# Varkalandar/raysnail

Hardware: AMD Instinct MI355X
Metric: Msamples/s (whole node) + ms/frame, RTIOW-13.1 scene 800x500x64spp (higher is better)
Workload: dtype f64; 1 GPU; rtow_13_1 balls_scene(seed 7)+light, 800x500, 64 spp, depth 8; width=800, height=500, spp=64, depth=8, split=rows, lanes=default, frames_in_flight=default, samples_per_frame=25600000

## Files before the change

raysnail_amd/csrc/rs_cam_cand.h:

```cpp
#pragma once
#include <math.h>
#include <stdint.h>

#if defined(__HIPCC__) || defined(__CUDACC__)
#define RS_CC_HD __host__ __device__
#else
#define RS_CC_HD
#endif

namespace rs {

constexpr uint32_t kCandMax = 8;
constexpr uint32_t kCandEmpty = 0xFFFFu;
constexpr uint32_t kCandOverflow = 0xFFFEu;
constexpr uint32_t kCandMaxEntries = 65534u;
constexpr int kCandStack = 32;

struct CandCam {
    double o[3];
    double lb[3], hf[3], vf[3];
    double R;
    double rho;
    double inv_w, inv_h, h;
    int ok;
// ... 33 lines not shown
    const double slack = 1.0 + 0x1p-40;
    c.R = fabs(aperture) * 0.5 * sqrt((hu2 > vu2 ? hu2 : vu2) + huvu) * slack;
    c.rho = sqrt(hf2 / (4.0 * w * w) + vf2 / (4.0 * h * h) + hfvf / (2.0 * w * h)) * slack;
    c.inv_w = 1.0 / w; c.inv_h = 1.0 / h; c.h = h;
    c.ok = cand_finite(c.R) && cand_finite(c.rho);
    return c;
}

RS_CC_HD inline CandBeam cand_beam(const CandCam& c, uint32_t x, uint32_t y) {
    CandBeam b;
    const double u = ((double)x + 0.5) * c.inv_w, v = (c.h - 1.5 - (double)y) * c.inv_h;
    double l2 = 0.0;
    for (int k = 0; k < 3; ++k) {
        b.o[k] = c.o[k];
        b.d[k] = c.lb[k] + u * c.hf[k] + v * c.vf[k] - c.o[k];
        l2 += b.d[k] * b.d[k];
    }
    b.len = sqrt(l2);
    b.inv_len = 1.0 / b.len;
    b.inv_len2 = 1.0 / l2;
    b.R = c.R; b.rho = c.rho;
    b.ok = c.ok && cand_finite(l2) && l2 > 0.0 && cand_finite(b.inv_len2);
    b.b[0] = c.rho - c.R;
    b.b[1] = c.R + c.rho;
    b.wide = 0;
    for (int piece = 0; piece < 2; ++piece) {
        const double k = b.b[piece] * b.inv_len;
        if (!(fabs(k) <= 0.99)) { b.wide = 1; b.kf[piece] = 0.0; continue; }
        b.kf[piece] = k * b.inv_len / sqrt(1.0 - k * k);
    }
    return b;
}

RS_CC_HD inline bool cand_sphere(const CandBeam& b, const double c[3], double r, double* along = nullptr) {
    const double w[3] = {c[0] - b.o[0], c[1] - b.o[1], c[2] - b.o[2]};
    const double w1 = fabs(w[0]) + fabs(w[1]) + fabs(w[2]);
    const double p = (w[0] * b.d[0] + w[1] * b.d[1] + w[2] * b.d[2]) * b.inv_len2;
    if (along) *along = p;
    if (!b.ok || b.wide) return true;
    r = fabs(r);
    const double reach = w1 + b.R + r;
    r = sqrt(r * r + 0x1p-40 * reach * reach);
    if (!(r - r == 0.0)) return true;
    const double cx = w[1] * b.d[2] - w[2] * b.d[1], cy = w[2] * b.d[0] - w[0] * b.d[2], cz = w[0] * b.d[1] - w[1] * b.d[0];
    const double h = sqrt(cx * cx + cy * cy + cz * cz) * b.inv_len;
    for (int piece = 0; piece < 2; ++piece) {
        const double bb = b.b[piece];
        const double aa = piece == 0 ? r + b.R : r - b.R;
        double s = p + h * b.kf[piece];
        if (piece == 0) s = s < 0.0 ? 0.0 : s > 1.0 ? 1.0 : s;
        else s = s < 1.0 ? 1.0 : s;
        if (!(s - s == 0.0)) return true;
        const double q[3] = {w[0] - s * b.d[0], w[1] - s * b.d[1], w[2] - s * b.d[2]};
        const double dist = sqrt(q[0] * q[0] + q[1] * q[1] + q[2] * q[2]);
        const double g = dist - (aa + bb * s);
        const double slack = 0x1p-30 * (w1 + r + b.R + s * (b.len + b.R + b.rho));
        if (!(g > slack)) return true;
    }
    return false;
}

struct CandList {
    uint32_t e[kCandMax];
    double along[kCandMax];
    uint32_t n;
};
// ... 18 lines not shown
```

raysnail_amd/csrc/rs_host.cpp:

```cpp
#include <hip/hip_runtime.h>

#include <algorithm>
#include <atomic>
#include <chrono>
#include <functional>
#include <cmath>
#include <cstdio>
#include <cstdlib>
#include <cstring>
#include <memory>
#include <new>
#include <stdexcept>
#include <string>
#include <vector>

#include "../../include/raysnail_hip.h"
#include "rs_host_util.h"
#include "rs_internal.h"
#include "rs_layout.h"

using namespace rs;

namespace {

// ... 670 lines not shown
    DScene& d = s->hs.ds;
    d.limg = nullptr;
    d.limg_bytes = 0;
    std::memset(d.limg_off, 0, sizeof(d.limg_off));
    if (s->scene_mode != kSmNest0 && s->scene_mode != kSmNest2) return;
    if (d.root4 < 0 || !d.ref_order || s->stack_need + (int)kLeafBatch > stack_lds(s->scene_mode)) return;
    const uint32_t cap = kLimgMax;
#ifdef RS_DEV_KNOBS
    if (std::getenv("RS_NO_LIMG")) return;
#endif
    const void* const* fields[LT_COUNT] = {
        (const void* const*)&d.nodes4, (const void* const*)&d.pbox, (const void* const*)&d.pclass,
        (const void* const*)&d.prims, (const void* const*)&d.spheres, (const void* const*)&d.rects,
        (const void* const*)&d.boxes, (const void* const*)&d.quadrics, (const void* const*)&d.csgs,
        (const void* const*)&d.xforms, (const void* const*)&d.tf_fwd, (const void* const*)&d.tf_inv};
    std::vector<char> img;
    for (int t = 0; t < LT_COUNT; ++t) {
        const size_t fo = (size_t)((const char*)fields[t] - (const char*)&d);
        img.resize((img.size() + 15) & ~(size_t)15);
        d.limg_off[t] = (uint32_t)img.size();
        for (const Blob& b : s->hs.blobs)
            if (b.field_off == fo) img.insert(img.end(), b.bytes.begin(), b.bytes.end());
        if (img.size() > cap) return;
    }
    img.resize((img.size() + 15) & ~(size_t)15);
    if (img.size() > cap) return;
    d.limg_bytes = (uint32_t)img.size();
    Blob b;
    b.field_off = (size_t)((const char*)&d.limg - (const char*)&d);
    b.bytes = std::move(img);
    s->hs.blobs.push_back(std::move(b));
}

void upload_replica(rs_scene* s, int device) {
    std::unique_ptr<Replica> R(new Replica());
    R->device = device;
    HIP_OK(hipSetDevice(device));
    R->ds = s->hs.ds;
    for (const Blob& b : s->hs.blobs) {
        void* p = nullptr;
        HIP_OK(hipMalloc(&p, b.bytes.size()));
        R->dev.push_back(p);
        HIP_OK(hipMemcpy(p, b.bytes.data(), b.bytes.size(), hipMemcpyHostToDevice));
        std::memcpy((char*)&R->ds + b.field_off, &p, sizeof(void*));
    }
    HIP_OK(hipMalloc((void**)&R->d_ds, sizeof(DScene)));
    std::memset(&R->uploaded, 0xff, sizeof(DScene));
    HIP_OK(hipStreamCreateWithFlags(&R->stream, hipStreamNonBlocking));
#ifdef RS_DEV_KNOBS
    if (const char* e = std::getenv("RS_PAD_STREAMS"))
        for (int k = std::atoi(e); k > 0; --k) {
            hipStream_t st;
            HIP_OK(hipStreamCreateWithFlags(&st, hipStreamNonBlocking));
            R->pad_streams.push_back(st);
        }
#endif
    hipDeviceProp_t prop;
    HIP_OK(hipGetDeviceProperties(&prop, device));
    R->n_cu = prop.multiProcessorCount;
    R->mem_total = (uint64_t)prop.totalGlobalMem;
    HIP_OK(wf_occupancy(s->scene_mode, &R->ext_bpc, &R->shade_bpc));
    s->reps.push_back(std::move(R));
}

void build(rs_scene* s) {
    if (s->committed) throw Error(RS_E_STATE, "scene already committed");
    s->hs = HostScene();
    for (uint32_t h : s->world) if (s->nest_depth(h) > RS_MAX_NEST) throw Error(RS_E_UNSUPPORTED, "object nesting deeper than the GPU path supports");
    for (uint32_t h : s->lights) if (s->nest_depth(h) > RS_MAX_NEST) throw Error(RS_E_UNSUPPORTED, "light nesting deeper than the GPU path supports");

    std::vector<DMaterial> mats;
    for (const rs_material_desc& d : s->mdesc) {
        DMaterial m;
        std::memset(&m, 0, sizeof(m));
        m.kind = d.kind; m.tex_kind = d.texture.kind; m.tex_data = d.texture.data; m.glass = d.glass;
        m.k_specular = d.k_specular;
        m.mix_a = d.mix_a; m.mix_b = d.mix_b;
        for (int i = 0; i < 4; ++i) { m.even[i] = d.texture.even[i]; m.odd[i] = d.texture.odd[i]; }
        m.tex_scale = d.texture.scale;
        m.enter_refractive = 1.0 / d.refractive;
        m.outer_refractive = d.refractive;
        m.exponent = d.exponent; m.multiplier = d.multiplier; m.mix_p = d.mix_p;
        const rs_material_desc* e = &d;
        for (int k = 0; k < 64 && e->kind == RS_MAT_MIXED; ++k) e = &s->mdesc[e->mix_a];
        m.phong_factor = e->phong_factor; m.phong_exponent = e->phong_exponent;
        mats.push_back(m);
    }
    DMaterial dm;
    std::memset(&dm, 0, sizeof(dm));
    dm.kind = RS_MAT_LAMBERTIAN; dm.tex_kind = RS_TEX_SOLID;
    for (int i = 0; i < 4; ++i) dm.even[i] = 1.0f;
    dm.enter_refractive = dm.outer_refractive = 1.0; dm.multiplier = 1.0; dm.phong_exponent = 1;
    const int32_t default_mat = (int32_t)mats.size();
    mats.push_back(dm);
// ... 279 lines not shown
            s->tree_depth = depth4;
            s->n_nodes = n4.size();
            s->stack_need = stack_need4_ref(n4, r4);
        }
    }
    d.stack_need = s->stack_need;
    d.moving = 0;
    for (const DSphere& sp : spheres)
        if (sp.v[0] != 0.0 || sp.v[1] != 0.0 || sp.v[2] != 0.0) d.moving = 1;
    d.stk_ovf = nullptr;
    stage(s, d.prims, prims);
    stage(s, d.spheres, spheres);
    stage(s, d.lprim, leaves.prims);
    s->n_leaf_entries = leaves.prims.size();
    if (s->scene_mode == kSmSpheres) {
        std::vector<DSphere> lsph(s->objs.size());
        std::memset(lsph.data(), 0, lsph.size() * sizeof(DSphere));
        for (size_t h = 0; h < s->objs.size(); ++h)
            if (s->objs[h].kind == PK_SPHERE) lsph[h] = spheres[prims[h].idx];
        if (lsph.size() * sizeof(DSphere) > 0xFFFFFFFFull) throw Error(RS_E_INVALID, "scene too large: sphere array over 4 GiB");
        if (d.moving) {
            stage(s, d.lsph, lsph);
        } else {
            std::vector<DSphereS> lsphs(lsph.size());
            for (size_t h = 0; h < lsph.size(); ++h) {
                for (int k = 0; k < 3; ++k) lsphs[h].c[k] = lsph[h].c[k];
                lsphs[h].r = lsph[h].r;
                if (s->objs[h].kind == PK_SPHERE && lsph[h].r * lsph[h].r != lsph[h].r2)
                    throw Error(RS_E_INVALID, "sphere radius_squared is not radius * radius");
            }
            stage(s, d.lsphs, lsphs);
        }
    }
    if (s->scene_mode == kSmFlat) {
        std::vector<LTri> ltri(leaves.prims.size());
        std::memset(ltri.data(), 0, ltri.size() * sizeof(LTri));
        for (size_t e = 0; e < ltri.size(); ++e) {
            const DPrim& P = prims[leaves.prims[e]];
            ltri[e].kind = (double)P.kind;
            if (P.kind != PK_TRIANGLE) continue;
            const DTri& T = tris[P.idx];
            for (int k = 0; k < 3; ++k) ltri[e].p0[k] = T.p0[k];
            ltri[e].a = T.a; ltri[e].b = T.b; ltri[e].c = T.c; ltri[e].d = T.d; ltri[e].e = T.e; ltri[e].f = T.f;
        }
        if (ltri.size() * sizeof(LTri) > 0xFFFFFFFFull) throw Error(RS_E_INVALID, "scene too large: leaf triangle array over 4 GiB");
        stage(s, d.ltri, ltri);
    }
    stage(s, d.rects, rects);
    stage(s, d.boxes, boxes);
    stage(s, d.quadrics, quads);
    stage(s, d.tris, tris);
    stage(s, d.csgs, csgs);
    stage(s, d.xforms, xforms);
    stage(s, d.tf_fwd, tf_f);
    stage(s, d.tf_inv, tf_i);
    stage(s, d.mats, mats);
    stage(s, d.media, media);
    d.has_media = media.empty() ? 0 : 1;
    std::vector<DPerlin> dper;
    std::vector<double> tf64;
    std::vector<int32_t> ti32;
    for (const HPerlin& hp : s->perlins) {
        DPerlin x;
        std::memset(&x, 0, sizeof(x));
        x.point_count = (int32_t)hp.d.point_count; x.vector = hp.d.vector; x.smooth = hp.d.smooth; x.type = hp.d.type;
        x.depth = (int32_t)hp.d.depth; x.scale = hp.d.scale;
// ... 1904 lines not shown
```

raysnail_amd/csrc/rs_internal.h:

```cpp
#pragma once
#include <hip/hip_runtime.h>
#include <stdint.h>
#include "rs_layout.h"
#include "rs_cam_cand.h"

namespace rs {

constexpr int kBlock = 256;
constexpr int kStackMax = 24;
constexpr int kStackMin = 16;
constexpr uint32_t kLeafBatch = 8;
constexpr uint32_t kMaxLanes = 4;
constexpr uint32_t kMaxSlots = 4;
constexpr int kMaxFrames = 64;

enum SceneMode { kSmGeneric = 0, kSmSpheres = 1, kSmFlat = 2, kSmNest0 = 3, kSmNest2 = 4, kSmMarch = 5 };
constexpr bool generic_mode(int sm) { return sm == kSmGeneric || sm == kSmMarch; }
constexpr int march_of(int sm) { return sm == kSmMarch ? 1 : 0; }
constexpr int nest_of(int sm) { return sm == kSmNest0 ? 0 : sm == kSmNest2 ? 2 : generic_mode(sm) ? RS_MAX_NEST : 0; }
constexpr int rich_of(int sm) { return generic_mode(sm) ? 1 : 0; }
constexpr bool streaming_mode(int sm) { return sm == kSmSpheres || sm == kSmNest0 || sm == kSmNest2; }
constexpr int stack_lds(int sm) { return generic_mode(sm) ? kStackMax : kStackMin; }
static_assert(4u * ((uint32_t)stack_lds(kSmNest0) * kBlock * 4u + kLimgMax) <= 160u * 1024u, "LDS image budget");
static_assert(4u * ((uint32_t)stack_lds(kSmNest2) * kBlock * 4u + kLimgMax) <= 160u * 1024u, "LDS image budget");

struct SceneRef {
    const DScene* host;
    const DScene* dev;
};
#if defined(RS_NO_FLAT_DYN) || defined(RS_TRAV_STATS)
inline bool flat_dyn(const SceneRef&) { return false; }
#else
inline bool flat_dyn(const SceneRef& s) { return s.host->root4 >= 0; }
#endif
#ifdef RS_NO_FLAT_LAMB
inline bool flat_lamb(const SceneRef&) { return false; }
#else
// ... 58 lines not shown
hipError_t launch_probe_shade(const SceneRef& s, const double* rows, uint32_t n, uint64_t key_base, double* out, int sm,
                              hipStream_t st);
hipError_t launch_probe_camera(const DCamera& c, const PathParams& p, const uint32_t* xys, uint32_t n, int centres,
                               double* out, int sm, hipStream_t st);
hipError_t launch_path_mega(const SceneRef& s, const DCamera& c, const PathParams& p, int sm, double* rad,
                            unsigned long long* seg_counters, uint32_t max_blocks, hipStream_t st);
hipError_t launch_wf_gen(const DCamera& c, const PathParams& p, const WfState& w, uint64_t item0, uint32_t n, double* rad,
                         hipStream_t st);
hipError_t launch_wf_extend(const SceneRef& s, const WfState& w, uint32_t bounce, uint32_t blocks, int sm, hipStream_t st);
hipError_t launch_wf_shade(const SceneRef& s, const WfState& w, uint32_t bounce, uint32_t depth, uint64_t n_items, double* rad,
                           uint32_t blocks, int sm, hipStream_t st);

constexpr int kWfsClasses = 5;
#ifndef RS_CNT_PAD
#define RS_CNT_PAD 32
#endif
constexpr uint32_t kCntPad = RS_CNT_PAD;
constexpr int kCntStat0 = 8;
constexpr uint32_t kStatLines = 8;
constexpr uint32_t kWfsStride = (kCntStat0 + kStatLines) * kCntPad;
__host__ __device__ constexpr uint32_t cix(int slot) { return (uint32_t)slot * kCntPad; }
constexpr int kCntFront = 6, kCntBack = 7;
constexpr int kExtAll = 0, kExtCarried = 1, kExtCamera = 2;
constexpr bool ext_split(int sm) { return sm == kSmNest2 || sm == kSmSpheres; }
#ifndef RS_CAM_FUSE
#define RS_CAM_FUSE 1
#endif
constexpr bool cam_fused(int sm, int part) { return RS_CAM_FUSE && sm == kSmSpheres && part == kExtCamera; }
#ifndef RS_CAM_CAND
#define RS_CAM_CAND 1
#endif
constexpr bool cam_cand(int sm, int part) { return RS_CAM_CAND && sm == kSmSpheres && part == kExtCamera; }
hipError_t launch_cam_cand_build(const SceneRef& s, const DCamera& c, const PathParams& p, uint4* cand, hipStream_t st);
hipError_t launch_wfs_extend(const SceneRef& s, const DCamera& c, const PathParams& p, const WfState& w,
                             QEnt* const* queues, uint32_t it, const InjParams& inj, double* rad, uint32_t blocks,
                             int part, int sm, hipStream_t st, hipEvent_t ev0 = nullptr, hipEvent_t ev1 = nullptr);
hipError_t launch_wfs_finish(const SceneRef& s, const WfState& w, uint32_t it, uint32_t depth, double* rad, uint32_t blocks,
                             int sm, hipStream_t st);
hipError_t launch_wfs_shade_all(const SceneRef& s, const WfState& w, QEnt* const* queues, uint32_t class_mask,
                                uint32_t it, uint32_t depth, double* rad, uint32_t blocks, bool split, int sm,
                                hipStream_t st);
hipError_t wf_occupancy(int sm, int* extend_blocks_per_cu, int* shade_blocks_per_cu);
hipError_t launch_combine(float* acc, const float* nw, uint64_t n, float p, hipStream_t st);
hipError_t launch_noise(const float* px, int w, int h, float t, uint8_t* redo, unsigned int* minmax_bits,
                        unsigned long long* count, hipStream_t st);
hipError_t launch_probe_hit(const SceneRef& s, const double* rays, uint32_t n, double tmin, double tmax, double* out, int sm,
                            hipStream_t st);
hipError_t launch_features(const SceneRef& s, const DCamera& c, const PathParams& p, uint32_t max_specular, float* out_albedo,
                           float* out_normal, unsigned long long* seg_counter, int sm, uint32_t max_blocks, hipStream_t st);
hipError_t launch_denoise(const float* beauty, const float* albedo, const float* normal, uint32_t width, uint32_t height,
                          uint32_t levels, const float* ic, float inv_n, float inv_d, int gamma, float* out, float* work,
                          hipStream_t st);
hipError_t launch_pass_moments(const float* const* frames, uint32_t n_frames, uint32_t n_pix, int gamma, float* mean,
                               float* var, hipStream_t st);
hipError_t launch_denoise_var(const float* beauty, const float* var, const float* albedo, const float* normal,
                              uint32_t width, uint32_t height, uint32_t levels, float k_color, float inv_n, float inv_d,
                              int gamma, float* out, float* out_var, float* work, hipStream_t st);
hipError_t launch_pass_robust(const float* const* frames, uint32_t n_frames, uint32_t n_pix, int gamma, float trim,
                              float* mean, float* var, uint8_t* trimmed, hipStream_t st);
hipError_t launch_moments_update(float* acc, float* m2, const float* const* frames, uint32_t n_frames, uint32_t n_pix,
                                 int gamma, hipStream_t st);
hipError_t launch_moments_resolve(const float* acc, const float* m2, uint32_t n_pix, int gamma, float* mean, float* var,
                                  hipStream_t st);
hipError_t launch_adaptive_mask(const float* acc, const float* m2, const uint8_t* base, uint32_t width, uint32_t height,
                                uint32_t min_n, uint32_t max_n, float tol2, float floor, uint32_t radius, uint8_t* mask,
                                unsigned int* counters, hipStream_t st, uint32_t row_begin, uint32_t row_end,
// ... 8 lines not shown
```

raysnail_amd/csrc/rs_kernels.hip:

```cpp
#include <cstdlib>
#include <type_traits>

#include <hip/hip_ext.h>

#include "rs_device.h"
#include "rs_internal.h"
#include "rs_gen_perm.h"

#define RS_PASTE_(a, b) a##b
#define RS_PASTE(a, b) RS_PASTE_(a, b)
#if !defined(RS_TU)
#define RS_TU_COMMON 1
#define RS_TU_MODES 1
#define RS_TU_SUFFIX
#elif RS_TU < 0
#define RS_TU_COMMON 1
#define RS_TU_MODES 0
#define RS_TU_SUFFIX _c
#elif RS_TU == 6
#define RS_TU_COMMON 0
#define RS_TU_MODES 0
#define RS_TU_SUFFIX _6
#else
#define RS_TU_COMMON 0
// ... 1265 lines not shown

constexpr int kClasses = kWfsClasses;
constexpr int kClsLight = 6;

constexpr int ext_min_waves(int sm, bool lobj = false, int part = kExtAll) {
    if (sm == kSmSpheres) return 5;
    return sm == kSmNest2 ? (lobj ? 3 : 2) : 4;
}

extern __shared__ uint4 s_limg[];
__device__ __forceinline__ void lds_fill(const DScene& Sv) {
    const uint32_t nq = Sv.limg_bytes >> 4;
    const uint4* __restrict__ src = (const uint4*)Sv.limg;
    for (uint32_t q = threadIdx.x; q < nq; q += kBlock) s_limg[q] = src[q];
    __syncthreads();
}
__device__ __forceinline__ void lds_scene(const DScene* __restrict__ Sp, DScene& Sv, bool fill = true) {
    Sv = *Sp;
    if (fill) lds_fill(Sv);
    const char* b = (const char*)s_limg;
    Sv.nodes4 = (const DNode4*)(b + Sv.limg_off[LT_NODES4]);
    Sv.pclass = (const uint8_t*)(b + Sv.limg_off[LT_PCLASS]);
    Sv.pbox = (const DBox64*)(b + Sv.limg_off[LT_PBOX]);
    Sv.prims = (const DPrim*)(b + Sv.limg_off[LT_PRIMS]);
    Sv.spheres = (const DSphere*)(b + Sv.limg_off[LT_SPHERES]);
    Sv.rects = (const DRect*)(b + Sv.limg_off[LT_RECTS]);
    Sv.boxes = (const DBox*)(b + Sv.limg_off[LT_BOXES]);
    Sv.quadrics = (const DQuadric*)(b + Sv.limg_off[LT_QUADRICS]);
    Sv.csgs = (const DCsg*)(b + Sv.limg_off[LT_CSGS]);
    Sv.xforms = (const DXform*)(b + Sv.limg_off[LT_XFORMS]);
    Sv.tf_fwd = (const DMat34*)(b + Sv.limg_off[LT_TF_FWD]);
    Sv.tf_inv = (const DMat34*)(b + Sv.limg_off[LT_TF_INV]);
}
template <int SM, bool OVF, int PART, bool LOBJ>
__global__ __launch_bounds__(kBlock, ext_min_waves(SM, LOBJ, PART)) void k_wfs_extend(const DScene* __restrict__ Sp, WfState W,
                                                                          QEnt* const* __restrict__ queues, uint32_t it,
                                                                          double* __restrict__ rad, DCamera C, PathParams P,
                                                                          InjParams I) {
    DScene Sv;
    if constexpr (LOBJ) lds_scene(Sp, Sv, false);
    const DScene& S = LOBJ ? Sv : *Sp;
    __shared__ int stk_all[stack_lds(SM) * kBlock];
    const StkT<OVF, stack_lds(SM)> stk = make_stk<OVF, stack_lds(SM)>(S, stk_all);
    constexpr bool kTop = SM == kSmSpheres && kLTop > 0;
    uint32_t* cnt = W.counts + (size_t)it * kWfsStride;
    const uint32_t nf = cnt[cix(kCntFront)];
    const uint32_t n_old = PART == kExtCamera ? 0u : nf + cnt[cix(kCntBack)];
    const uint32_t n = n_old + (PART == kExtCarried ? 0u : I.n_new);
    if (PART != kExtCamera && blockIdx.x == 0 && threadIdx.x == 0) cnt[0] = n_old;
    const WfSet& cur = W.set[it & 1];
    constexpr bool kFuse = cam_fused(SM, PART);
    constexpr bool kCand = cam_cand(SM, PART);
    const uint32_t base0 = blockIdx.x * kBlock;
    for (uint32_t base = base0; base < n; base += gridDim.x * kBlock) {
        const uint32_t j = base + threadIdx.x;
        const bool gen = PART == kExtCamera || (PART == kExtAll && j >= n_old);
        const uint32_t i = gen ? nf + (j - n_old) : j < nf ? j : W.cap - 1u - (j - nf);
        int cls = -1, qbp = 0;
        int fcls = -1;
        double qt = 0.0;
        bool live = false;
        Ray r;
        Rng rng;
        uint32_t item = 0;
        [[maybe_unused]] uint32_t pl = 0;
        if (j < n) {
            if (gen) {
                uint64_t g, key;
                inj_sample(I, P, j - n_old, g, key, item);
                live = camera_sample(C, P, key, g, r, rng, kCand ? &pl : nullptr);
                if (!live) put_rad(rad, item, 0.0, 0.0, 0.0);
            } else {
                r = load_ray(cur, i, W.tagw);
                live = true;
            }
        }
        if constexpr (LOBJ)
            if (base == base0) lds_fill(S);
        if constexpr (kTop)
            if (base == base0) {
                const uint32_t nq = (uint32_t)S.ltop * (sizeof(DNode4) / 16);
                const uint4* __restrict__ src = (const uint4*)S.nodes4;
                for (uint32_t q = threadIdx.x; q < nq; q += kBlock) ((uint4*)s_top4)[q] = src[q];
                __syncthreads();
            }
        if (live) {
            double bend = RS_INF;
            constexpr bool kT = SM == kSmSpheres;
            int bp = -1;
            bool walk = true;
            if constexpr (kCand) {
                if (I.cand) {
                    const i4v rv = gld<i4v>(I.cand, pl * 16u);
                    uint4 rec = make_uint4((uint32_t)rv.x, (uint32_t)rv.y, (uint32_t)rv.z, (uint32_t)rv.w);
                    if ((rec.x & 0xFFFFu) != kCandOverflow) {
                        const RayC rc = ray_consts(r);
                        double best = RS_INF, be = RS_INF;
                        bool tie = false;
                        TravStat st;
                        for (uint32_t k = 0; k < kCandMax; ++k) {
                            const uint32_t e = rec.x & 0xFFFFu;
                            if (e == kCandEmpty) break;
                            rec.x = (rec.x >> 16) | (rec.y << 16); rec.y = (rec.y >> 16) | (rec.z << 16);
                            rec.z = (rec.z >> 16) | (rec.w << 16); rec.w = (rec.w >> 16) | 0xFFFF0000u;
                            st.leaf();
                            test_sphere_leaf<true>(S, ld_sphere_s(S.lsphs, (int)e), (int)e, r, rc, 0.0001, best, be, bp, &tie);
                        }
                        if (!tie) {
                            walk = false;
                            st.store();
                            bend = best;
                            if (bp >= 0 && S.lprim) bp = S.lprim[bp];
                        }
                    }
                }
            }
            if (walk) bp = traverse<SM, StkT<OVF, stack_lds(SM)>, LOBJ, kT, kTop>(S, r, 0.0001, bend, stk);
            V3 add;
            bool done = true;
            if (bp < 0) {
                add = background(S, r);
            } else {
                cls = (int)S.pclass[bp];
                if (cls == kClsLight) {
                    Hit h;
                    int mi;
                    if (SM == kSmSpheres) {
                        const DPrim Pr = S.prims[bp];
                        sphere_rec_at(S.spheres[Pr.idx], Pr.mat, r, bend, h);
                        mi = Pr.mat;
                    } else {
                        if (S.prims[bp].kind != PK_XFORM) {
                            HitT ht;
                            Obj<0, 0>::hit_t(S, bp, r, 0.0001, bend, ht);
                            h.p = ht.p;
                            mi = S.prims[bp].mat;
                        } else {
                            finish_hit<SM, true>(S, bp, r, 0.0001, bend, h);
                            mi = h.mat;
                        }
                    }
                    add = emission<0>(S, S.mats[mi >= 0 ? mi : S.default_mat], h);
                    cls = -1;
                } else {
                    qbp = bp;
                    qt = bend;
                    if (kFuse && (cls == 0 || cls == 1 || cls == 3)) {
                        fcls = cls;
// ... 684 lines not shown
                                  float* out_albedo, float* out_normal, unsigned long long* seg_counter,
                                  uint32_t max_blocks, hipStream_t st) {
    const uint32_t N = p.sqrt_spp * p.sqrt_spp;
    const uint32_t ppw = 64 / (N < 64 ? (N ? N : 1u) : 64u);
    const uint64_t groups = ((uint64_t)p.n_pix_local + ppw - 1) / ppw;
    const uint64_t blocks = std::min<uint64_t>((groups + kBlock / 64 - 1) / (kBlock / 64), max_blocks);
    if (!blocks) return hipSuccess;
    if (max_specular == 0)
        hipLaunchKernelGGL(k_features<SM>, dim3((uint32_t)blocks), dim3(kBlock), 0, st, s.dev, c, p,
                           reinterpret_cast<float4*>(out_albedo), reinterpret_cast<float4*>(out_normal), seg_counter);
    else
        hipLaunchKernelGGL(k_features_spec<SM>, dim3((uint32_t)blocks), dim3(kBlock), 0, st, s.dev, c, p, max_specular,
                           reinterpret_cast<float4*>(out_albedo), reinterpret_cast<float4*>(out_normal), seg_counter);
    return hipGetLastError();
}
#if !defined(RS_TU) || RS_TU == 5
hipError_t features_march(const SceneRef& s, const DCamera& c, const PathParams& p, uint32_t max_specular, float* out_albedo,
                          float* out_normal, unsigned long long* seg_counter, uint32_t max_blocks, hipStream_t st) {
    return features_launch<kSmMarch>(s, c, p, max_specular, out_albedo, out_normal, seg_counter, max_blocks, st);
}
#endif
#if !defined(RS_TU) || RS_TU == 6
hipError_t features_march(const SceneRef& s, const DCamera& c, const PathParams& p, uint32_t max_specular, float* out_albedo,
                          float* out_normal, unsigned long long* seg_counter, uint32_t max_blocks, hipStream_t st);
hipError_t launch_features(const SceneRef& s, const DCamera& c, const PathParams& p, uint32_t max_specular, float* out_albedo,
                           float* out_normal, unsigned long long* seg_counter, int sm, uint32_t max_blocks, hipStream_t st) {
    if (sm == kSmMarch) return features_march(s, c, p, max_specular, out_albedo, out_normal, seg_counter, max_blocks, st);
    return features_launch<kSmGeneric>(s, c, p, max_specular, out_albedo, out_normal, seg_counter, max_blocks, st);
}
#endif
#endif

#if !defined(RS_TU) || RS_TU == 1
__global__ __launch_bounds__(kBlock) void k_cam_cand_build(const DScene* __restrict__ Sp, DCamera C, PathParams P,
                                                           uint4* __restrict__ cand) {
    const uint32_t pl = blockIdx.x * kBlock + threadIdx.x;
    if (pl >= P.n_pix_local) return;
    const DScene& S = *Sp;
    const uint32_t x = pl % P.width, y = P.row_begin + (pl / P.width) * P.row_step;
    const CandCam cc = cand_camera(C.origin, C.lb, C.hf, C.vf, C.hu, C.vu, C.aperture, P.width, P.height);
    const CandBeam b = cand_beam(cc, x, y);
    CandList l;
    cand_list_init(l);
    if (!b.ok || S.root4 < 0) {
        l.n = kCandMax + 1;
    } else {
        int stk[kCandStack];
        int sp = 0, node = S.root4;
        while (node >= 0 && !cand_list_overflow(l)) {
            const DNode4& N = S.nodes4[node];
            int next = -1;
            for (int k = 0; k < 4; ++k) {
                const int c = N.child[k];
                if (c == INT32_MIN) continue;
                const double lo[3] = {(double)N.lo_x[k], (double)N.lo_y[k], (double)N.lo_z[k]};
                const double hi[3] = {(double)N.hi_x[k], (double)N.hi_y[k], (double)N.hi_z[k]};
                const double ctr[3] = {0.5 * (lo[0] + hi[0]), 0.5 * (lo[1] + hi[1]), 0.5 * (lo[2] + hi[2])};
                const double ex = hi[0] - lo[0], ey = hi[1] - lo[1], ez = hi[2] - lo[2];
                const double rad = 0.5 * sqrt(ex * ex + ey * ey + ez * ez) * (1.0 + 0x1p-40);
                if (!cand_sphere(b, ctr, rad)) continue;
                if (c < 0) {
                    const DSphere sp_ = ld_sphere_s(S.lsphs, ~c);
                    double along;
                    if (cand_sphere(b, sp_.c, sp_.r, &along)) cand_list_add(l, (uint32_t)~c, along);
                } else if (next < 0) {
                    next = c;
                } else if (sp < kCandStack) {
                    stk[sp++] = c;
                } else {
                    l.n = kCandMax + 1;
                }
            }
            if (next < 0 && sp > 0) next = stk[--sp];
            node = next;
        }
    }
    uint32_t w[4];
    cand_list_pack(l, w);
    cand[pl] = make_uint4(w[0], w[1], w[2], w[3]);
}

hipError_t launch_cam_cand_build(const SceneRef& s, const DCamera& c, const PathParams& p, uint4* cand, hipStream_t st) {
    const uint32_t blocks = (p.n_pix_local + kBlock - 1) / kBlock;
    if (!blocks) return hipSuccess;
    hipLaunchKernelGGL(k_cam_cand_build, dim3(blocks), dim3(kBlock), 0, st, s.dev, c, p, cand);
    return hipGetLastError();
}
#endif

#define RS_SM_LAUNCHERS(X)                                                                                     \
    X(hipError_t, probe_sample, (const SceneRef& s, const DCamera& c, const PathParams& p, uint32_t x, uint32_t y,  \
                                 uint32_t s0, uint32_t n, double* out, hipStream_t st), (s, c, p, x, y, s0, n, out, st)) \
    X(hipError_t, path_mega, (const SceneRef& s, const DCamera& c, const PathParams& p, double* rad,              \
                              unsigned long long* seg_counters, uint32_t max_blocks, hipStream_t st),             \
      (s, c, p, rad, seg_counters, max_blocks, st))                                                            \
    X(hipError_t, wf_extend, (const SceneRef& s, const WfState& w, uint32_t bounce, uint32_t blocks, hipStream_t st), \
      (s, w, bounce, blocks, st))                                                                              \
    X(hipError_t, wf_shade, (const SceneRef& s, const WfState& w, uint32_t bounce, uint32_t depth, uint64_t n_items,  \
                             double* rad, uint32_t blocks, hipStream_t st), (s, w, bounce, depth, n_items, rad, blocks, st)) \
    X(hipError_t, wf_occupancy, (int* e, int* sh), (e, sh))                                                    \
    X(hipError_t, probe_shade, (const SceneRef& s, const double* rows, uint32_t n, uint64_t key_base, double* out,  \
                                hipStream_t st), (s, rows, n, key_base, out, st))                               \
    X(hipError_t, probe_camera, (const DCamera& c, const PathParams& p, const uint32_t* xys, uint32_t n, int centres, \
                                 double* out, hipStream_t st), (c, p, xys, n, centres, out, st))
#define RS_SORTED_LAUNCHERS(X)                                                                                 \
    X(hipError_t, wfs_extend, (const SceneRef& s, const DCamera& c, const PathParams& p, const WfState& w,       \
                               QEnt* const* queues, uint32_t it, const InjParams& inj, double* rad, uint32_t blocks, \
                               int part, hipStream_t st, hipEvent_t ev0, hipEvent_t ev1),                        \
      (s, c, p, w, queues, it, inj, rad, blocks, part, st, ev0, ev1))                                                  \
    X(hipError_t, wfs_finish, (const SceneRef& s, const WfState& w, uint32_t it, uint32_t depth, double* rad,        \
                               uint32_t blocks, hipStream_t st), (s, w, it, depth, rad, blocks, st))              \
    X(hipError_t, wfs_shade_all, (const SceneRef& s, const WfState& w, QEnt* const* queues, uint32_t class_mask, \
// ... 287 lines not shown
```

raysnail_amd/csrc/rs_layout.h:

```cpp
#pragma once
#include <stdint.h>

#define RS_MAX_NEST 4

namespace rs {

enum PrimKind : int32_t {
    PK_SPHERE = 0,
    PK_RECT = 1,
    PK_BOX = 2,
    PK_QUADRIC = 3,
    PK_TRIANGLE = 4,
    PK_AND = 5,
    PK_SUB = 6,
    PK_XFORM = 7,
    PK_MEDIUM = 8,
    PK_RAYMARCH = 9,
};

struct DPrim {
    int32_t kind;
    int32_t idx;
    int32_t mat;
    int32_t aux;
};

struct DSphere {
    double c[3];
    double r;
    double r2;
    double v[3];
};

struct alignas(32) DSphereS {
// ... 115 lines not shown
    const LTri* ltri;
    const DRect* rects;
    const DBox* boxes;
    const DQuadric* quadrics;
    const DTri* tris;
    const DCsg* csgs;
    const DXform* xforms;
    const DMat34* tf_fwd;
    const DMat34* tf_inv;
    const DMaterial* mats;
    const DMedium* media;
    const DPerlin* perlins;
    const DImage* images;
    const double* tex_f64;
    const int32_t* tex_i32;
    const uint8_t* tex_u8;
    const int32_t* lights;
    int32_t* stk_ovf;
    const void* limg;
    uint32_t limg_bytes;
    uint32_t limg_off[LT_COUNT];
    int32_t n_lights;
    int32_t root;
    int32_t default_mat;
    int32_t ref_order;
    int32_t root4;
    int32_t uv;
    int32_t has_media;
    int32_t stack_need;
    int32_t moving;
    int32_t ltop;
    int32_t lamb_only;
    float bg_lo[4], bg_hi[4];
};

#ifndef RS_LTOP
#define RS_LTOP 85
#endif
constexpr int kLTop = RS_LTOP;


struct DCamera {
    double origin[3], lb[3], hf[3], vf[3], hu[3], vu[3];
    double aperture, shutter;
};

}
```

Baseline: 5138 Msamples/s.

## Add precomputed light-directed candidate grid to skip BVH traversal for light rays

Builds a uniform 3D grid over the sphere scene. For each cell, a conservative beam (cell ball toward the single spherical light) is walked through the BVH once at upload, storing up to eight candidate spheres per cell. During extension of carried (bounce) rays whose origin cell is valid and whose direction points into the light's cone, only the candidate list is tested instead of a full traversal. It falls back to traversal on overflow or ties. This adds a per-ray membership test, grid memory and a build kernel, and only helps rays aimed at the light.

```diff
diff --git a/raysnail_amd/csrc/rs_cam_cand.h b/raysnail_amd/csrc/rs_cam_cand.h
--- a/raysnail_amd/csrc/rs_cam_cand.h
+++ b/raysnail_amd/csrc/rs_cam_cand.h
@@ -89,6 +89,32 @@
     return b;
 }
 
+RS_CC_HD inline CandBeam cand_beam_ball(const double O[3], double R, const double F[3], double rho) {
+    CandBeam b;
+    double l2 = 0.0;
+    bool fin = cand_finite(R) && cand_finite(rho);
+    for (int k = 0; k < 3; ++k) {
+        b.o[k] = O[k];
+        b.d[k] = F[k] - O[k];
+        l2 += b.d[k] * b.d[k];
+        fin = fin && cand_finite(O[k]) && cand_finite(F[k]);
+    }
+    b.len = sqrt(l2);
+    b.inv_len = 1.0 / b.len;
+    b.inv_len2 = 1.0 / l2;
+    b.R = fabs(R); b.rho = fabs(rho);
+    b.ok = fin && cand_finite(l2) && l2 > 0.0 && cand_finite(b.inv_len2);
+    b.b[0] = b.rho - b.R;
+    b.b[1] = b.R + b.rho;
+    b.wide = 0;
+    for (int piece = 0; piece < 2; ++piece) {
+        const double k = b.b[piece] * b.inv_len;
+        if (!(fabs(k) <= 0.99)) { b.wide = 1; b.kf[piece] = 0.0; continue; }
+        b.kf[piece] = k * b.inv_len / sqrt(1.0 - k * k);
+    }
+    return b;
+}
+
 RS_CC_HD inline bool cand_sphere(const CandBeam& b, const double c[3], double r, double* along = nullptr) {
     const double w[3] = {c[0] - b.o[0], c[1] - b.o[1], c[2] - b.o[2]};
     const double w1 = fabs(w[0]) + fabs(w[1]) + fabs(w[2]);
diff --git a/raysnail_amd/csrc/rs_host.cpp b/raysnail_amd/csrc/rs_host.cpp
--- a/raysnail_amd/csrc/rs_host.cpp
+++ b/raysnail_amd/csrc/rs_host.cpp
@@ -726,6 +726,13 @@
     s->hs.blobs.push_back(std::move(b));
 }
 
+bool light_cand_scene(const rs_scene* s, const DScene& d) {
+    return light_cand(s->scene_mode, kExtCarried) && d.moving == 0 && d.root4 >= 0 && !s->ref_order &&
+           s->objs.size() <= kCandMaxEntries && s->stack_need <= kCandStack && s->lights.size() == 1;
+}
+
+bool try_malloc(void** p, size_t bytes);
+
 void upload_replica(rs_scene* s, int device) {
     std::unique_ptr<Replica> R(new Replica());
     R->device = device;
@@ -754,6 +761,17 @@
     R->n_cu = prop.multiProcessorCount;
     R->mem_total = (uint64_t)prop.totalGlobalMem;
     HIP_OK(wf_occupancy(s->scene_mode, &R->ext_bpc, &R->shade_bpc));
+    if (R->ds.lgrid.cells) {
+        void* p = nullptr;
+        if (R->ds.lsphs && try_malloc(&p, (size_t)R->ds.lgrid.cells * sizeof(uint4))) {
+            R->dev.push_back(p);
+            R->ds.lcand = (const uint32_t*)p;
+            HIP_OK(launch_light_cand_build(R->ref(), (uint4*)p, R->stream));
+            HIP_OK(hipStreamSynchronize(R->stream));
+        } else {
+            R->ds.lgrid.cells = 0;
+        }
+    }
     s->reps.push_back(std::move(R));
 }
 
@@ -1099,6 +1117,20 @@
             stage(s, d.lsphs, lsphs);
         }
     }
+    d.lgrid = LightGrid{};
+    d.lcand = nullptr;
+    if (light_cand_scene(s, d) && lights.size() == 1 && s->objs[lights[0]].kind == PK_SPHERE) {
+        std::vector<double> c, r;
+        uint32_t light = 0;
+        for (size_t h = 0; h < s->objs.size(); ++h) {
+            if (s->objs[h].kind != PK_SPHERE) continue;
+            if ((int32_t)h == lights[0]) light = (uint32_t)r.size();
+            const DSphere& sp = spheres[prims[h].idx];
+            c.insert(c.end(), sp.c, sp.c + 3);
+            r.push_back(sp.r);
+        }
+        d.lgrid = light_grid_make(c.data(), r.data(), (uint32_t)r.size(), light);
+    }
     if (s->scene_mode == kSmFlat) {
         std::vector<LTri> ltri(leaves.prims.size());
         std::memset(ltri.data(), 0, ltri.size() * sizeof(LTri));
diff --git a/raysnail_amd/csrc/rs_internal.h b/raysnail_amd/csrc/rs_internal.h
--- a/raysnail_amd/csrc/rs_internal.h
+++ b/raysnail_amd/csrc/rs_internal.h
@@ -3,6 +3,7 @@
 #include <stdint.h>
 #include "rs_layout.h"
 #include "rs_cam_cand.h"
+#include "rs_light_cand.h"
 
 namespace rs {
 
@@ -127,6 +128,11 @@
 #endif
 constexpr bool cam_cand(int sm, int part) { return RS_CAM_CAND && sm == kSmSpheres && part == kExtCamera; }
 hipError_t launch_cam_cand_build(const SceneRef& s, const DCamera& c, const PathParams& p, uint4* cand, hipStream_t st);
+#ifndef RS_LIGHT_CAND
+#define RS_LIGHT_CAND 1
+#endif
+constexpr bool light_cand(int sm, int part) { return RS_LIGHT_CAND && sm == kSmSpheres && part == kExtCarried; }
+hipError_t launch_light_cand_build(const SceneRef& s, uint4* cand, hipStream_t st);
 hipError_t launch_wfs_extend(const SceneRef& s, const DCamera& c, const PathParams& p, const WfState& w,
                              QEnt* const* queues, uint32_t it, const InjParams& inj, double* rad, uint32_t blocks,
                              int part, int sm, hipStream_t st, hipEvent_t ev0 = nullptr, hipEvent_t ev1 = nullptr);
diff --git a/raysnail_amd/csrc/rs_kernels.hip b/raysnail_amd/csrc/rs_kernels.hip
--- a/raysnail_amd/csrc/rs_kernels.hip
+++ b/raysnail_amd/csrc/rs_kernels.hip
@@ -1321,6 +1321,28 @@
     Sv.tf_fwd = (const DMat34*)(b + Sv.limg_off[LT_TF_FWD]);
     Sv.tf_inv = (const DMat34*)(b + Sv.limg_off[LT_TF_INV]);
 }
+__device__ __forceinline__ bool cand_list_hit(const DScene& S, uint4 rec, const Ray& r, int& bp, double& t) {
+    if ((rec.x & 0xFFFFu) == kCandOverflow) return false;
+    const RayC rc = ray_consts(r);
+    double best = RS_INF, be = RS_INF;
+    int b = -1;
+    bool tie = false;
+    TravStat st;
+    for (uint32_t k = 0; k < kCandMax; ++k) {
+        const uint32_t e = rec.x & 0xFFFFu;
+        if (e == kCandEmpty) break;
+        rec.x = (rec.x >> 16) | (rec.y << 16); rec.y = (rec.y >> 16) | (rec.z << 16);
+        rec.z = (rec.z >> 16) | (rec.w << 16); rec.w = (rec.w >> 16) | 0xFFFF0000u;
+        st.leaf();
+        test_sphere_leaf<true>(S, ld_sphere_s(S.lsphs, (int)e), (int)e, r, rc, 0.0001, best, be, b, &tie);
+    }
+    if (tie) return false;
+    st.store();
+    t = best;
+    bp = (b >= 0 && S.lprim) ? S.lprim[b] : b;
+    return true;
+}
+
 template <int SM, bool OVF, int PART, bool LOBJ>
 __global__ __launch_bounds__(kBlock, ext_min_waves(SM, LOBJ, PART)) void k_wfs_extend(const DScene* __restrict__ Sp, WfState W,
                                                                           QEnt* const* __restrict__ queues, uint32_t it,
@@ -1340,6 +1362,7 @@
     const WfSet& cur = W.set[it & 1];
     constexpr bool kFuse = cam_fused(SM, PART);
     constexpr bool kCand = cam_cand(SM, PART);
+    constexpr bool kLCand = light_cand(SM, PART);
     const uint32_t base0 = blockIdx.x * kBlock;
     for (uint32_t base = base0; base < n; base += gridDim.x * kBlock) {
         const uint32_t j = base + threadIdx.x;
@@ -1381,28 +1404,25 @@
             if constexpr (kCand) {
                 if (I.cand) {
                     const i4v rv = gld<i4v>(I.cand, pl * 16u);
-                    uint4 rec = make_uint4((uint32_t)rv.x, (uint32_t)rv.y, (uint32_t)rv.z, (uint32_t)rv.w);
-                    if ((rec.x & 0xFFFFu) != kCandOverflow) {
-                        const RayC rc = ray_consts(r);
-                        double best = RS_INF, be = RS_INF;
-                        bool tie = false;
-                        TravStat st;
-                        for (uint32_t k = 0; k < kCandMax; ++k) {
-                            const uint32_t e = rec.x & 0xFFFFu;
-                            if (e == kCandEmpty) break;
-                            rec.x = (rec.x >> 16) | (rec.y << 16); rec.y = (rec.y >> 16) | (rec.z << 16);
-                            rec.z = (rec.z >> 16) | (rec.w << 16); rec.w = (rec.w >> 16) | 0xFFFF0000u;
-                            st.leaf();
-                            test_sphere_leaf<true>(S, ld_sphere_s(S.lsphs, (int)e), (int)e, r, rc, 0.0001, best, be, bp, &tie);
-                        }
-                        if (!tie) {
-                            walk = false;
-                            st.store();
-                            bend = best;
-                            if (bp >= 0 && S.lprim) bp = S.lprim[bp];
-                        }
+                    walk = !cand_list_hit(S, make_uint4((uint32_t)rv.x, (uint32_t)rv.y, (uint32_t)rv.z, (uint32_t)rv.w), r, bp, bend);
+                }
+            }
+            if constexpr (kLCand) {
+                if (j < nf && S.lcand) {
+                    const double o[3] = {r.o.x, r.o.y, r.o.z}, d[3] = {r.d.x, r.d.y, r.d.z};
+                    const uint32_t cell = light_cell(S.lgrid, o);
+                    if (cell != kLightOutside && light_member(S.lgrid, o, d)) {
+                        const i4v rv = gld<i4v>(S.lcand, cell * 16u);
+                        walk = !cand_list_hit(S, make_uint4((uint32_t)rv.x, (uint32_t)rv.y, (uint32_t)rv.z, (uint32_t)rv.w), r, bp, bend);
                     }
                 }
+#ifdef RS_TRAV_STATS
+                if (j < nf) {
+                    if (!walk) { atomicAdd(&g_trav_stats[1][24], 1ull); atomicAdd(&g_trav_stats[1][25], (unsigned long long)s_st_leaves[threadIdx.x]); }
+                    const unsigned long long wm = __ballot(walk);
+                    if (wm && (threadIdx.x & 63) == (unsigned)(__ffsll((long long)__ballot(1)) - 1)) atomicAdd(&g_trav_stats[1][26], 1ull);
+                }
+#endif
             }
             if (walk) bp = traverse<SM, StkT<OVF, stack_lds(SM)>, LOBJ, kT, kTop>(S, r, 0.0001, bend, stk);
             V3 add;
@@ -2153,6 +2173,43 @@
 #endif
 
 #if !defined(RS_TU) || RS_TU == 1
+__device__ __forceinline__ void cand_beam_walk(const DScene& S, const CandBeam& b, CandList& l) {
+    cand_list_init(l);
+    if (!b.ok || S.root4 < 0) {
+        l.n = kCandMax + 1;
+        return;
+    }
+    int stk[kCandStack];
+    int sp = 0, node = S.root4;
+    while (node >= 0 && !cand_list_overflow(l)) {
+        const DNode4& N = S.nodes4[node];
+        int next = -1;
+        for (int k = 0; k < 4; ++k) {
+            const int c = N.child[k];
+            if (c == INT32_MIN) continue;
+            const double lo[3] = {(double)N.lo_x[k], (double)N.lo_y[k], (double)N.lo_z[k]};
+            const double hi[3] = {(double)N.hi_x[k], (double)N.hi_y[k], (double)N.hi_z[k]};
+            const double ctr[3] = {0.5 * (lo[0] + hi[0]), 0.5 * (lo[1] + hi[1]), 0.5 * (lo[2] + hi[2])};
+            const double ex = hi[0] - lo[0], ey = hi[1] - lo[1], ez = hi[2] - lo[2];
+            const double rad = 0.5 * sqrt(ex * ex + ey * ey + ez * ez) * (1.0 + 0x1p-40);
+            if (!cand_sphere(b, ctr, rad)) continue;
+            if (c < 0) {
+                const DSphere sp_ = ld_sphere_s(S.lsphs, ~c);
+                double along;
+                if (cand_sphere(b, sp_.c, sp_.r, &along)) cand_list_add(l, (uint32_t)~c, along);
+            } else if (next < 0) {
+                next = c;
+            } else if (sp < kCandStack) {
+                stk[sp++] = c;
+            } else {
+                l.n = kCandMax + 1;
+            }
+        }
+        if (next < 0 && sp > 0) next = stk[--sp];
+        node = next;
+    }
+}
+
 __global__ __launch_bounds__(kBlock) void k_cam_cand_build(const DScene* __restrict__ Sp, DCamera C, PathParams P,
                                                            uint4* __restrict__ cand) {
     const uint32_t pl = blockIdx.x * kBlock + threadIdx.x;
@@ -2162,43 +2219,28 @@
     const CandCam cc = cand_camera(C.origin, C.lb, C.hf, C.vf, C.hu, C.vu, C.aperture, P.width, P.height);
     const CandBeam b = cand_beam(cc, x, y);
     CandList l;
-    cand_list_init(l);
-    if (!b.ok || S.root4 < 0) {
-        l.n = kCandMax + 1;
-    } else {
-        int stk[kCandStack];
-        int sp = 0, node = S.root4;
-        while (node >= 0 && !cand_list_overflow(l)) {
-            const DNode4& N = S.nodes4[node];
-            int next = -1;
-            for (int k = 0; k < 4; ++k) {
-                const int c = N.child[k];
-                if (c == INT32_MIN) continue;
-                const double lo[3] = {(double)N.lo_x[k], (double)N.lo_y[k], (double)N.lo_z[k]};
-                const double hi[3] = {(double)N.hi_x[k], (double)N.hi_y[k], (double)N.hi_z[k]};
-                const double ctr[3] = {0.5 * (lo[0] + hi[0]), 0.5 * (lo[1] + hi[1]), 0.5 * (lo[2] + hi[2])};
-                const double ex = hi[0] - lo[0], ey = hi[1] - lo[1], ez = hi[2] - lo[2];
-                const double rad = 0.5 * sqrt(ex * ex + ey * ey + ez * ez) * (1.0 + 0x1p-40);
-                if (!cand_sphere(b, ctr, rad)) continue;
-                if (c < 0) {
-                    const DSphere sp_ = ld_sphere_s(S.lsphs, ~c);
-                    double along;
-                    if (cand_sphere(b, sp_.c, sp_.r, &along)) cand_list_add(l, (uint32_t)~c, along);
-                } else if (next < 0) {
-                    next = c;
-                } else if (sp < kCandStack) {
-                    stk[sp++] = c;
-                } else {
-                    l.n = kCandMax + 1;
-                }
-            }
-            if (next < 0 && sp > 0) next = stk[--sp];
-            node = next;
-        }
-    }
+    cand_beam_walk(S, b, l);
     uint32_t w[4];
     cand_list_pack(l, w);
     cand[pl] = make_uint4(w[0], w[1], w[2], w[3]);
+}
+
+__global__ __launch_bounds__(kBlock) void k_light_cand_build(const DScene* __restrict__ Sp, uint4* __restrict__ cand) {
+    const DScene& S = *Sp;
+    const uint32_t cell = blockIdx.x * kBlock + threadIdx.x;
+    if (cell >= S.lgrid.cells) return;
+    CandList l;
+    cand_beam_walk(S, light_cell_beam(S.lgrid, cell), l);
+    uint32_t w[4];
+    cand_list_pack(l, w);
+    cand[cell] = make_uint4(w[0], w[1], w[2], w[3]);
+}
+
+hipError_t launch_light_cand_build(const SceneRef& s, uint4* cand, hipStream_t st) {
+    const uint32_t blocks = (s.host->lgrid.cells + kBlock - 1) / kBlock;
+    if (!blocks) return hipSuccess;
+    hipLaunchKernelGGL(k_light_cand_build, dim3(blocks), dim3(kBlock), 0, st, s.dev, cand);
+    return hipGetLastError();
 }
 
 hipError_t launch_cam_cand_build(const SceneRef& s, const DCamera& c, const PathParams& p, uint4* cand, hipStream_t st) {
diff --git a/raysnail_amd/csrc/rs_layout.h b/raysnail_amd/csrc/rs_layout.h
--- a/raysnail_amd/csrc/rs_layout.h
+++ b/raysnail_amd/csrc/rs_layout.h
@@ -1,5 +1,6 @@
 #pragma once
 #include <stdint.h>
+#include "rs_light_cand.h"
 
 #define RS_MAX_NEST 4
 
@@ -181,6 +182,8 @@
     int32_t ltop;
     int32_t lamb_only;
     float bg_lo[4], bg_hi[4];
+    LightGrid lgrid;
+    const uint32_t* lcand;
 };
 
 #ifndef RS_LTOP
diff --git a/raysnail_amd/csrc/rs_light_cand.h b/raysnail_amd/csrc/rs_light_cand.h
--- /dev/null
+++ b/raysnail_amd/csrc/rs_light_cand.h
@@ -0,0 +1,124 @@
+#pragma once
+#include "rs_cam_cand.h"
+
+namespace rs {
+
+constexpr uint32_t kLightOutside = 0xFFFFFFFFu;
+constexpr uint32_t kLightCellsMax = 1u << 17;
+
+struct LightGrid {
+    double lo[3];
+    double inv;
+    double h;
+    double f[3];
+    double rho;
+    double rho2m;
+    double grow;
+    uint32_t n[3];
+    uint32_t cells;
+};
+
+RS_CC_HD inline uint32_t light_cell(const LightGrid& g, const double o[3]) {
+    if (g.cells == 0) return kLightOutside;
+    uint32_t idx[3];
+    for (int k = 0; k < 3; ++k) {
+        const double q = (o[k] - g.lo[k]) * g.inv;
+        if (!(q >= 0.0 && q < (double)g.n[k])) return kLightOutside;
+        idx[k] = (uint32_t)q;
+    }
+    return (idx[2] * g.n[1] + idx[1]) * g.n[0] + idx[0];
+}
+
+RS_CC_HD inline void light_cell_ball(const LightGrid& g, uint32_t cell, double O[3], double* R) {
+    const uint32_t idx[3] = {cell % g.n[0], (cell / g.n[0]) % g.n[1], cell / (g.n[0] * g.n[1])};
+    for (int k = 0; k < 3; ++k) O[k] = g.lo[k] + ((double)idx[k] + 0.5) * g.h;
+    *R = 0.8660254037844387 * g.h * (1.0 + 0x1p-20) + g.grow;
+}
+
+RS_CC_HD inline CandBeam light_cell_beam(const LightGrid& g, uint32_t cell) {
+    double O[3], R;
+    light_cell_ball(g, cell, O, &R);
+    return cand_beam_ball(O, R, g.f, g.rho);
+}
+
+RS_CC_HD inline bool light_member(const LightGrid& g, const double o[3], const double d[3]) {
+    const double w[3] = {g.f[0] - o[0], g.f[1] - o[1], g.f[2] - o[2]};
+    const double ahead = w[0] * d[0] + w[1] * d[1] + w[2] * d[2];
+    const double cx = w[1] * d[2] - w[2] * d[1], cy = w[2] * d[0] - w[0] * d[2], cz = w[0] * d[1] - w[1] * d[0];
+    const double d2 = d[0] * d[0] + d[1] * d[1] + d[2] * d[2];
+    return ahead > 0.0 && cx * cx + cy * cy + cz * cz <= g.rho2m * d2;
+}
+
+inline LightGrid light_grid_make(const double* c, const double* r, uint32_t n, uint32_t light,
+                                 uint32_t max_cells = kLightCellsMax) {
+    LightGrid g;
+    g.cells = 0; g.inv = g.h = g.rho = g.rho2m = g.grow = 0.0;
+    for (int k = 0; k < 3; ++k) { g.lo[k] = g.f[k] = 0.0; g.n[k] = 0; }
+    if (n < 2 || light >= n) return g;
+    double med;
+    {
+        double* t = new double[n];
+        for (uint32_t i = 0; i < n; ++i) t[i] = fabs(r[i]);
+        for (uint32_t i = 0; i <= n / 2; ++i) {
+            uint32_t m = i;
+            for (uint32_t j = i + 1; j < n; ++j) if (t[j] < t[m]) m = j;
+            const double x = t[i]; t[i] = t[m]; t[m] = x;
+        }
+        med = t[n / 2];
+        delete[] t;
+    }
+    if (!(med > 0.0) || !cand_finite(med)) return g;
+    double lo[3] = {INFINITY, INFINITY, INFINITY}, hi[3] = {-INFINITY, -INFINITY, -INFINITY};
+    for (uint32_t i = 0; i < n; ++i) {
+        const double ri = fabs(r[i]);
+        if (!cand_finite(ri) || !cand_finite(c[3 * i]) || !cand_finite(c[3 * i + 1]) || !cand_finite(c[3 * i + 2])) return g;
+        if (!(ri <= 16.0 * med)) continue;
+        for (int k = 0; k < 3; ++k) {
+            if (c[3 * i + k] - ri < lo[k]) lo[k] = c[3 * i + k] - ri;
+            if (c[3 * i + k] + ri > hi[k]) hi[k] = c[3 * i + k] + ri;
+        }
+    }
+    double ext[3], vol = 1.0;
+    for (int k = 0; k < 3; ++k) {
+        ext[k] = hi[k] - lo[k];
+        if (!(ext[k] > 0.0) || !cand_finite(ext[k]) || !cand_finite(lo[k])) return g;
+        vol *= ext[k];
+    }
+    if (max_cells == 0 || max_cells > kLightCellsMax) max_cells = kLightCellsMax;
+    double h = cbrt(vol / (double)max_cells);
+    if (h < 0.5 * med) h = 0.5 * med;
+    for (int it = 0; it < 400; ++it, h *= 1.01) {
+        double cells = 1.0;
+        for (int k = 0; k < 3; ++k) cells *= ceil(ext[k] / h) + 2.0;
+        if (cells <= (double)max_cells) break;
+    }
+    double cells = 1.0, M = 0.0;
+    for (int k = 0; k < 3; ++k) {
+        const double nk = ceil(ext[k] / h) + 2.0;
+        cells *= nk;
+        if (!(nk >= 1.0 && nk <= (double)kLightCellsMax)) return g;
+        g.n[k] = (uint32_t)nk;
+        g.lo[k] = lo[k] - h;
+        const double a = fabs(g.lo[k]), b = fabs(g.lo[k] + nk * h);
+        if (a > M) M = a;
+        if (b > M) M = b;
+    }
+    if (!(cells <= (double)kLightCellsMax) || !cand_finite(h) || !cand_finite(M)) return g;
+    g.h = h;
+    g.inv = 1.0 / h;
+    g.grow = 0x1p-20 * M;
+    g.rho = fabs(r[light]);
+    g.rho2m = g.rho * g.rho * (1.0 - 0x1p-20);
+    double far2 = 0.0;
+    for (int k = 0; k < 3; ++k) {
+        g.f[k] = c[3 * light + k];
+        const double a = fabs(g.f[k] - g.lo[k]), b = fabs(g.f[k] - (g.lo[k] + (double)g.n[k] * h));
+        far2 += (a > b ? a : b) * (a > b ? a : b);
+    }
+    if (!(g.rho > 0.0) || !cand_finite(g.rho) || !cand_finite(far2) || !(far2 <= 0x1p24 * g.rho * g.rho)) return g;
+    if (!cand_finite(g.inv)) return g;
+    g.cells = g.n[0] * g.n[1] * g.n[2];
+    return g;
+}
+
+}
```

Result: faster. 5303 Msamples/s (median of 6 runs) (+3.2%).
